# showlab/VideoSwap

Measured on AMD Instinct MI355X. Metric: denoised frames/sec, 16-frame 512x512 clip @ 50 DDIM steps (end to end: inversion + CFG sampling), higher is better.
Workload: dtype f16; 1 GPU; BASELINE.json configs[1]: 16-frame 512x512 clip, SD-1.5 UNet3D + AnimateDiff motion modules, 50-step DDIM inversion (B=1) + 50-step CFG-7.5 DDIM sampling (B=2), 1 clip per GPU per step; launch=eager, parallelism=clip-parallel x1

## Files before the change

videoswap_amd/build.py:

```python
import hashlib
import os
import re
import shutil
import subprocess
import sys
import tempfile
from concurrent.futures import ThreadPoolExecutor

HERE = os.path.dirname(os.path.abspath(__file__))
ROOT = os.path.dirname(HERE)
CSRC = os.path.join(HERE, 'csrc')
LIBDIR = os.path.join(HERE, 'lib')
OBJDIR = os.path.join(LIBDIR, 'obj')
LIB = os.path.join(LIBDIR, 'libvsx.so')
VARIANTS = {}
VARIANT_EXTRA = {}
SOURCES = ['api.cpp', 'comm.cpp', 'options.cpp', 'prof.cpp', 'gemm.hip', 'gemm_pp.hip', 'norm.hip', 'attention.hip', 'attention_bwd.hip', 'elementwise.hip',
           'train.hip', 'dift.hip', 'atlas.hip', 'atlas_edit.hip']
HIPCC = os.environ.get('HIPCC', '/opt/rocm/bin/hipcc')
FLAGS = ['--offload-arch=gfx950', '-O3', '-std=c++17', '-fPIC', '-x', 'hip',
         '-I', os.path.join(ROOT, 'include'), '-I', CSRC, '-Wall', '-Wno-unused-function', '-Wno-division-by-zero',
         '-mllvm', '-amdgpu-mfma-vgpr-form']


def lib_path(variant=None):
    return LIB if not variant else os.path.join(LIBDIR, f'libvsx_{variant}.so')


def _digest(variant=None):
    h = hashlib.sha256()
    swap = VARIANTS[variant] if variant else {}
    names = [n for n in sorted(os.listdir(CSRC)) if n.endswith(('.hip', '.cpp', '.h'))]
    for name in names + ['../../include/vsx.h']:
        with open(os.path.join(CSRC, swap.get(name, name)), 'rb') as f:
            h.update(name.encode() + b'\0' + f.read())
    h.update(' '.join(f.replace(ROOT, '<root>') for f in FLAGS).encode())
    if variant:
        for name in VARIANT_EXTRA.get(variant, []):
            with open(os.path.join(CSRC, name), 'rb') as f:
                h.update(name.encode() + b'\0' + f.read())
        h.update(b'\0variant ' + variant.encode())
    return h.hexdigest()


def source_digest(variant=None):
    return _digest(variant)


_MARKER = b'@vsx-source-digest:'


def built_digest(variant=None):
    path = lib_path(variant)
    if not os.path.exists(path):
        return None
    with open(path, 'rb') as f:
        blob = f.read()
    i = blob.find(_MARKER)
    if i < 0:
        return None
    j = blob.find(b'\0', i)
    return blob[i + len(_MARKER):j].decode(errors='replace')


def _compile(src, digest, variant=None):
    objdir = OBJDIR if not variant else os.path.join(LIBDIR, f'obj_{variant}')
    os.makedirs(objdir, exist_ok=True)
    obj = os.path.join(objdir, src.replace('/', '_') + '.o')
    extra = [f'-DVSX_SOURCE_DIGEST="{digest}"'] if src == 'api.cpp' else []
    path = os.path.join(CSRC, (VARIANTS[variant] if variant else {}).get(src, src))
    cmd = [HIPCC] + FLAGS + extra + ['-c', path, '-o', obj]
    r = subprocess.run(cmd, capture_output=True, text=True)
    if r.returncode != 0:
        raise RuntimeError(f'hipcc failed for {src}:\n{r.stdout}\n{r.stderr}')
    if r.stderr.strip():
        sys.stderr.write(r.stderr)
    return obj


LLVM_BIN = os.environ.get('VSX_LLVM_BIN', '/opt/rocm/lib/llvm/bin')
NO_SCRATCH = ('gemm_pp_kernel', 'gemm_ws320_kernel', 'flash_attn_kernel', 'gemm_kernelILi256E', 'coord_mlp_kernel')


def parse_kernel_notes(text):
    keys = ('vgpr_count', 'agpr_count', 'sgpr_count', 'vgpr_spill_count', 'sgpr_spill_count',
            'private_segment_fixed_size', 'group_segment_fixed_size')
    out, cur = {}, None
    for line in text.splitlines():
        m = re.match(r'^\s+(-\s+)?\.(\w+):\s*(\S.*)?$', line)
        if not m:
            continue
        if m.group(1) and re.match(r'^  - ', line):
            cur = {}
        if cur is None:
            continue
        key, val = m.group(2), (m.group(3) or '').strip()
        if key == 'name' and re.match(r'^    \.name:', line):
            out[val] = cur
        elif key in keys and re.match(r'^  (- |  )\.', line):
            cur[key] = int(val)
    return out


def kernel_resources(lib=None):
    lib = lib or LIB
    objdump, readelf = os.path.join(LLVM_BIN, 'llvm-objdump'), os.path.join(LLVM_BIN, 'llvm-readelf')
    tmp = tempfile.mkdtemp(prefix='vsx_co_')
    try:
        copy = os.path.join(tmp, 'lib.so')
        shutil.copy(lib, copy)
        r = subprocess.run([objdump, '--offloading', copy], capture_output=True, text=True, cwd=tmp)
        if r.returncode != 0:
            raise RuntimeError(f'llvm-objdump --offloading failed:\n{r.stderr}')
        res = {}
        for name in sorted(os.listdir(tmp)):
            if 'gfx950' not in name:
                continue
            r = subprocess.run([readelf, '--notes', os.path.join(tmp, name)], capture_output=True, text=True)
            if r.returncode != 0:
                raise RuntimeError(f'llvm-readelf --notes failed on {name}:\n{r.stderr}')
            res.update(parse_kernel_notes(r.stdout))
        return res
    finally:
        shutil.rmtree(tmp, ignore_errors=True)


def demangle(names):
    filt = shutil.which('c++filt') or shutil.which('llvm-cxxfilt')
    out = []
    if filt and names:
        r = subprocess.run([filt], input='\n'.join(names), capture_output=True, text=True)
        out = r.stdout.splitlines() if r.returncode == 0 else []
    return dict(zip(names, out if len(out) == len(names) else names))


def scratch_offenders(resources, patterns=NO_SCRATCH):
    pretty = demangle(list(resources))
    bad = []
    for name, r in resources.items():
        if not any(p in name for p in patterns):
            continue
        if r.get('vgpr_spill_count', 0) or r.get('private_segment_fixed_size', 0):
            bad.append((pretty[name], r.get('vgpr_spill_count', 0), r.get('private_segment_fixed_size', 0)))
    return sorted(bad)


def check_no_scratch(lib=None):
    res = kernel_resources(lib)
    if not res:
        raise RuntimeError('no kernel metadata found in ' + (lib or LIB))
    bad = scratch_offenders(res)
    if bad:
        raise RuntimeError('kernels that must not use scratch do:\n' + '\n'.join(
            f'  {n}: {s} VGPRs spilled, {b} B private segment' for n, s, b in bad))
    return res


def build(force=False, verbose=True, variant=None):
    os.makedirs(OBJDIR, exist_ok=True)
    lib = lib_path(variant)
    digest = _digest(variant)
    if not force and built_digest(variant) == digest:
        if verbose:
            print(f'[vsx] {lib} is up to date')
# ... 96 lines not shown
```

videoswap_amd/csrc/attention.hip:

```cpp
#include "common.h"
#include "options.h"

#include <type_traits>

namespace {

struct AttnParams {
    const half_t* Q;
    const half_t* K;
    const half_t* VT;
    half_t* O;
    int nq, nk, heads;
    long ldq, ldk, ldvt, ldo;
    long q_bs, k_bs, vt_bs, o_bs;
    int kv_div;
    float scale_log2e;
    float* lse;
    long lse_ld;
};

#ifdef VSX_GEMM_TIMING
__device__ long* g_attn_dbg = nullptr;
#define ASTAMP(i) do { const long t_now = (long)clock64(); t_seg[i] += t_now - t_last; t_last = t_now; } while (0)
#else
#define ASTAMP(i) do { } while (0)
#endif

constexpr int KV_TILE = 64;
constexpr int VSTR = 72;
typedef __attribute__((address_space(3))) void* lds_ptr_t;

template <int D, int QB = 1, bool O16 = false>
__global__ __launch_bounds__(256) void flash_attn_kernel(const AttnParams p) {
    static_assert(!O16 || (QB == 1 && D % 16 != 0 && D <= 48), "16-row O tiles: one query block per wave, a spare padding row");
    constexpr int DK = (D + 15) / 16;
    constexpr int DT = (D + 31) / 32;
    constexpr int CT = (D + 15) / 16;
    constexpr int VROWS = O16 ? CT * 16 : DT * 32;
    constexpr int KSTR = DK * 16 + 8;
    constexpr bool HAS_SPARE = (VROWS > D);
    constexpr int KSPR = KSTR / 8, VSPR = VSTR / 8;
    constexpr int K_UNITS = KV_TILE * KSPR, V_UNITS = D * VSPR;
    constexpr int NKI = (K_UNITS + 255) / 256, NVI = (V_UNITS + 255) / 256;
    constexpr int K_BYTES = KV_TILE * KSTR * 2;
    constexpr int V_BYTES = VROWS * VSTR * 2;
    constexpr int STAGE = K_BYTES + V_BYTES;
    constexpr int OOB_OFF = (int)0x80000000;

    __shared__ __attribute__((aligned(16))) unsigned char smem[2 * STAGE];

    const int tid = threadIdx.x;
    const int lane = tid & 63;
    const int wave = __builtin_amdgcn_readfirstlane(tid >> 6);
    const int l31 = lane & 31, hi = lane >> 5;
    int wg = blockIdx.x;
    {
        const int nwg = gridDim.x, qq = nwg >> 3, rr = nwg & 7;
        const int xcd = wg & 7, local = wg >> 3;
        wg = (xcd < rr ? xcd * (qq + 1) : rr * (qq + 1) + (xcd - rr) * qq) + local;
    }
    constexpr int QTILE = 128 * QB;
    const int qtiles = (p.nq + QTILE - 1) / QTILE;
    const int qt = wg % qtiles;
    const int h = (wg / qtiles) % p.heads;
    const long b = wg / (qtiles * p.heads);
    const long kvb = b / p.kv_div;

    const int q0 = qt * QTILE + wave * (32 * QB) + l31;

    h8 qf[QB][DK];
#pragma unroll
    for (int x = 0; x < QB; ++x) {
        const int q = q0 + 32 * x;
        const bool qok = q < p.nq;
        const half_t* qrow = p.Q + b * p.q_bs + (long)(qok ? q : 0) * p.ldq + h * D;
#pragma unroll
        for (int t = 0; t < DK; ++t) {
            const int d0 = t * 16 + hi * 8;
            qf[x][t] = (qok && d0 < D) ? as_h8(ld16(qrow + d0)) : as_h8(make_uint4(0, 0, 0, 0));
        }
    }

    const half_t* Kb = p.K + kvb * p.k_bs + h * D;
    const half_t* Vb = p.VT + kvb * p.vt_bs + (long)h * D * p.ldvt;
    const __amdgpu_buffer_rsrc_t rsrcK = __builtin_amdgcn_make_buffer_rsrc(
        const_cast<half_t*>(Kb), 0, (int)((((long)p.nk - 1) * p.ldk + D) * 2), 0x00020000);
    const __amdgpu_buffer_rsrc_t rsrcV = __builtin_amdgcn_make_buffer_rsrc(
        const_cast<half_t*>(Vb), 0, (int)((long)D * p.ldvt * 2), 0x00020000);
    int vk[NKI], vv[NVI];
#pragma unroll
    for (int i = 0; i < NKI; ++i) {
        const int u = (wave * NKI + i) * 64 + lane;
        const int row = u / KSPR, slot = u - row * KSPR;
        const int key = (row & ~12) | ((row & 4) << 1) | ((row & 8) >> 1);
        vk[i] = (u < K_UNITS && slot * 8 < D) ? (int)(((long)key * p.ldk + slot * 8) * 2) : OOB_OFF;
    }
#pragma unroll
    for (int i = 0; i < NVI; ++i) {
        const int u = (wave * NVI + i) * 64 + lane;
        const int row = u / VSPR, slot = u - row * VSPR;
        vv[i] = (u < V_UNITS && slot < 8) ? (int)(((long)row * p.ldvt + slot * 8) * 2) : OOB_OFF;
    }
    for (int i = tid; i < 2 * (VROWS - D) * VSTR; i += 256) {
        const int st = i / ((VROWS - D) * VSTR), r = i - st * ((VROWS - D) * VSTR);
        const int row = D + r / VSTR, col = r - (r / VSTR) * VSTR;
        half_t* sv = reinterpret_cast<half_t*>(smem + st * STAGE + K_BYTES);
        sv[row * VSTR + col] = (HAS_SPARE && row == VROWS - 1 && col < KV_TILE) ? (half_t)1.f : (half_t)0.f;
    }

    auto issue = [&](int j0, int stage) {
        unsigned char* sb = smem + stage * STAGE;
        const int soffK = (int)((long)j0 * p.ldk * 2);
        const int soffV = j0 * 2;
// ... 160 lines not shown
                h8 pf[QB];
#pragma unroll
                for (int x = 0; x < QB; ++x) {
#pragma unroll
                    for (int jj = 0; jj < 8; ++jj) pf[x][jj] = (half_t)s[x][kt][8 * s2 + jj];
                }
                const int c0 = kt * 32 + 16 * s2 + 8 * hi;
#pragma unroll
                for (int t = 0; t < DT; ++t) {
                    const h8 vf = *reinterpret_cast<const h8*>(sV + (t * 32 + l31) * VSTR + c0);
#pragma unroll
                    for (int x = 0; x < QB; ++x) o[x][t] = __builtin_amdgcn_mfma_f32_32x32x16_f16(vf, pf[x], o[x][t], 0, 0, 0);
                }
            }
        }
        ASTAMP(5);
        stage ^= 1;
    };
    {
        int j0 = 0;
        for (; j0 + KV_TILE <= p.nk; j0 += KV_TILE) tile(j0, std::false_type{});
        if (j0 < p.nk) tile(j0, std::true_type{});
    }

#ifdef VSX_GEMM_TIMING
    if (lane == 0 && g_attn_dbg) {
        long* o_dbg = g_attn_dbg + ((long)blockIdx.x * 4 + wave) * 6;
        for (int k = 0; k < 6; ++k) o_dbg[k] = t_seg[k];
    }
#endif
    if constexpr (O16) {
        const int l15 = lane & 15, g = lane >> 4;
#pragma unroll
        for (int qt = 0; qt < 2; ++qt) {
            const float den = __shfl(o16[CT - 1][qt][3], 48 + l15, 64);
            const int q = (q0 - l31) + 16 * qt + l15;
            if (q < p.nq) {
                const float inv = 1.0f / den;
                half_t* orow = p.O + b * p.o_bs + (long)q * p.ldo + h * D;
#pragma unroll
                for (int t = 0; t < CT; ++t) {
                    const int c = t * 16 + 4 * g;
                    if (c < D) {
                        h4 pk;
#pragma unroll
                        for (int e = 0; e < 4; ++e) pk[e] = (half_t)(o16[t][qt][e] * inv);
                        *reinterpret_cast<h4*>(orow + c) = pk;
                    }
                }
            }
        }
        return;
    }
#pragma unroll
    for (int x = 0; x < QB; ++x) {
        if (HAS_SPARE) {
            constexpr int reg = 15;
            constexpr int owner_hi = 1;
            const float mine = o[x][DT - 1][reg];
            const float other = __shfl_xor(mine, 32, 64);
            l_i[x] = (hi == owner_hi) ? mine : other;
        }
        const int q = q0 + 32 * x;
        if (q < p.nq) {
            if (p.lse && hi == 0) p.lse[(b * p.heads + h) * p.lse_ld + q] = m_i[x] + __log2f(l_i[x]);
            const float inv = 1.0f / l_i[x];
            half_t* orow = p.O + b * p.o_bs + (long)q * p.ldo + h * D;
#pragma unroll
            for (int t = 0; t < DT; ++t)
#pragma unroll
                for (int g = 0; g < 4; ++g) {
                    const int c = t * 32 + 8 * g + 4 * hi;
                    if (c < D) {
                        h4 pk;
#pragma unroll
                        for (int e = 0; e < 4; ++e) pk[e] = (half_t)(o[x][t][4 * g + e] * inv);
                        *reinterpret_cast<h4*>(orow + c) = pk;
                    }
                }
        }
    }
}

template <int D>
int launch_attn(const AttnParams& p, long nb, hipStream_t stream) {
    if constexpr (D == 40 || D == 80) {
        const long wg2 = ((p.nq + 255) / 256) * (long)p.heads * nb;
        const long force = vsxg::gemm_option("attn_qb");
        if (force == 2 || (force == 0 && D == 80 && wg2 >= 512 && p.nq >= 256)) {
            hipLaunchKernelGGL((flash_attn_kernel<D, 2>), dim3((unsigned)wg2), dim3(256), 0, stream, p);
            return vsx_check_launch("vsx_attention_f16");
        }
    }
    dim3 grid((unsigned)(((p.nq + 127) / 128) * (long)p.heads * nb));
    if constexpr (D == 40) {
        if (p.lse == nullptr && vsxg::gemm_option("attn_o16") != 0) {
            hipLaunchKernelGGL((flash_attn_kernel<D, 1, true>), grid, dim3(256), 0, stream, p);
            return vsx_check_launch("vsx_attention_f16");
        }
    }
    hipLaunchKernelGGL((flash_attn_kernel<D, 1>), grid, dim3(256), 0, stream, p);
    return vsx_check_launch("vsx_attention_f16");
}

struct TempParams {
    const half_t* Q;
    const half_t* K;
    const half_t* V;
    half_t* O;
    int fq, fk, hw, heads, d;
    long ldq, ldkv, ldo;
    float scale;
    int direct_out;
};

__global__ __launch_bounds__(256) void temporal_attn_kernel(const TempParams p) {
    extern __shared__ __attribute__((aligned(16))) unsigned char smem_raw[];
    const int d = p.d, fq = p.fq, fk = p.fk;
    const int wave = threadIdx.x >> 6;
    const size_t slice = (((size_t)(fq + 2 * fk) * d * sizeof(half_t) + (size_t)fq * fk * sizeof(float)) + 15) & ~(size_t)15;
    unsigned char* base = smem_raw + wave * slice;
    half_t* sQ = reinterpret_cast<half_t*>(base);
    half_t* sK = sQ + fq * d;
    half_t* sV = sK + fk * d;
    float* sS = reinterpret_cast<float*>(sV + fk * d);

    const int lane = threadIdx.x & 63;
    const long site = blockIdx.x;
    const int h = min((int)blockIdx.y * 4 + wave, p.heads - 1);
    const long b = blockIdx.z;
    const int dv = d >> 3;

    constexpr int UB = 4;
    for (int i0 = lane; i0 < fq * dv; i0 += 64 * UB) {
        uint4 r[UB];
#pragma unroll
        for (int u = 0; u < UB; ++u) {
            const int i = i0 + 64 * u;
            if (i < fq * dv) {
                const int f = i / dv, c = (i - f * dv) * 8;
                r[u] = ld16(p.Q + ((b * fq + f) * p.hw + site) * p.ldq + h * d + c);
            }
        }
#pragma unroll
        for (int u = 0; u < UB; ++u) {
            const int i = i0 + 64 * u;
            if (i < fq * dv) {
                const int f = i / dv, c = (i - f * dv) * 8;
                st16(sQ + f * d + c, r[u]);
            }
        }
    }
    for (int i0 = lane; i0 < fk * dv; i0 += 64 * UB) {
        uint4 rk[UB], rv[UB];
#pragma unroll
        for (int u = 0; u < UB; ++u) {
            const int i = i0 + 64 * u;
            if (i < fk * dv) {
                const int f = i / dv, c = (i - f * dv) * 8;
                const long row = (b * fk + f) * p.hw + site;
                rk[u] = ld16(p.K + row * p.ldkv + h * d + c);
                rv[u] = ld16(p.V + row * p.ldkv + h * d + c);
            }
        }
#pragma unroll
        for (int u = 0; u < UB; ++u) {
// ... 123 lines not shown
#pragma unroll
    for (int r = 0; r < 16; ++r) {
        const int key = (r & 3) + 4 * ((r >> 2) & 1) + 8 * hi + 16 * (r >> 3);
        const bool v = qok && key >= lo && key < up;
        sc[r] = v ? sc[r] * sl2 : -INFINITY;
        mx = fmaxf(mx, sc[r]);
    }
    mx = fmaxf(mx, __shfl_xor(mx, 32, 64));
    if (mx == -INFINITY) mx = 0.f;
    float sum = 0.f;
#pragma unroll
    for (int r = 0; r < 16; ++r) {
        sc[r] = __builtin_amdgcn_exp2f(sc[r] - mx);
        sum += sc[r];
    }
    sum += __shfl_xor(sum, 32, 64);
    const float inv = sum > 0.f ? 1.0f / sum : 0.f;

    f16v o[DT];
#pragma unroll
    for (int t = 0; t < DT; ++t) o[t] = zero;
#pragma unroll
    for (int s2 = 0; s2 < 2; ++s2) {
        h8 pf;
#pragma unroll
        for (int jj = 0; jj < 8; ++jj) pf[jj] = (half_t)sc[8 * s2 + jj];
#pragma unroll
        for (int t = 0; t < DT; ++t) {
            const h8 vf = *reinterpret_cast<const h8*>(sVT + (t * 32 + l31) * VSTR + vt_col(16 * s2 + 8 * hi, (t * 32 + l31) >> 3));
            o[t] = __builtin_amdgcn_mfma_f32_32x32x16_f16(vf, pf, o[t], 0, 0, 0);
        }
    }
    if (p.direct_out) {
        if (qok) {
            half_t* orow = p.O + ((b * fq + qf_) * p.hw + site) * p.ldo + (long)(head0 + qg) * D;
#pragma unroll
            for (int t = 0; t < DT; ++t)
#pragma unroll
                for (int g4 = 0; g4 < 4; ++g4) {
                    const int c = t * 32 + 8 * g4 + 4 * hi;
                    if (c < D) {
                        h4 pk;
#pragma unroll
                        for (int e = 0; e < 4; ++e) pk[e] = (half_t)(o[t][4 * g4 + e] * inv);
                        *reinterpret_cast<h4*>(orow + c) = pk;
                    }
                }
        }
        return;
    }
    constexpr int OSTR = D + 4;
    static_assert(32 * OSTR <= DT * 32 * VSTR, "the staged output fits the wave's V^T tile");
    static_assert((D / 2 + 2) % 4 == 2, "staged row pitch");
    half_t* sO = sVT;
    __builtin_amdgcn_sched_barrier(0);
#pragma unroll
    for (int t = 0; t < DT; ++t)
#pragma unroll
        for (int g4 = 0; g4 < 4; ++g4) {
            const int c = t * 32 + 8 * g4 + 4 * hi;
            if (c < D) {
                h4 pk;
#pragma unroll
                for (int e = 0; e < 4; ++e) pk[e] = (half_t)(o[t][4 * g4 + e] * inv);
                *reinterpret_cast<h4*>(sO + l31 * OSTR + c) = pk;
            }
        }
    __builtin_amdgcn_sched_barrier(0);
    const int per_frame = G * DV;
    const int total = fq * per_frame;
#pragma unroll
    for (int i = 0; i < NVL; ++i) {
        const int u = lane + 64 * i;
        if (u < total) {
            const int f = u / per_frame, rem = u - f * per_frame;
            const int g = rem / DV, ch = rem - g * DV;
            if (head0 + g < p.heads) {
                const half_t* src = sO + (g * fq + f) * OSTR + ch * 8;
                const h4 lo4 = *reinterpret_cast<const h4*>(src), up4 = *reinterpret_cast<const h4*>(src + 4);
                const h8 v = {lo4[0], lo4[1], lo4[2], lo4[3], up4[0], up4[1], up4[2], up4[3]};
                st16(p.O + ((b * fq + f) * p.hw + site) * p.ldo + (long)(head0 + g) * D + ch * 8, as_u4(v));
            }
        }
    }
}

template <int D>
__global__ __launch_bounds__(256) void temporal_attn_mfma_long_kernel(const TempParams p) {
    constexpr int DK = (D + 15) / 16;
    constexpr int DT = (D + 31) / 32;
    constexpr int DV = D / 8;
    constexpr int VSTR = 40;
    constexpr int NVL = (32 * DV + 63) / 64;
    constexpr int NKB = 4;
    __shared__ __attribute__((aligned(16))) half_t smem[4][DT * 32 * VSTR];

    const int lane = threadIdx.x & 63;
    const int wave = threadIdx.x >> 6;
    const int l31 = lane & 31, hi = lane >> 5;
    const int fq = p.fq, fk = p.fk;
    const int G = 32 / fq;
    const int nkb = (fk + 31) >> 5;
    const long site = blockIdx.x;
    const long b = blockIdx.z;
    const int head0 = ((int)blockIdx.y * 4 + wave) * G;
    if (head0 >= p.heads) return;
    half_t* sVT = smem[wave];

    const int qg = l31 / fq, qf_ = l31 - qg * fq;
    const bool qok = qg < G && head0 + qg < p.heads;
    const half_t* qptr = p.Q + ((b * fq + qf_) * p.hw + site) * p.ldq + (long)(head0 + qg) * D + hi * 8;
    h8 qb[DK];
#pragma unroll
    for (int t = 0; t < DK; ++t)
        qb[t] = (qok && t * 16 + hi * 8 < D) ? as_h8(ld16(qptr + t * 16)) : as_h8(make_uint4(0, 0, 0, 0));

    const f16v zero = {0.f, 0.f, 0.f, 0.f, 0.f, 0.f, 0.f, 0.f, 0.f, 0.f, 0.f, 0.f, 0.f, 0.f, 0.f, 0.f};
    f16v sc[NKB];
#pragma unroll
    for (int kb = 0; kb < NKB; ++kb) sc[kb] = zero;
    const int krow = (l31 & ~12) | ((l31 & 4) << 1) | ((l31 & 8) >> 1);
    for (int g = 0; g < G; ++g) {
        if (head0 + g >= p.heads) break;
#pragma unroll
        for (int kb = 0; kb < NKB; ++kb) {
            if (kb >= nkb) continue;
            const int key = kb * 32 + krow;
            const half_t* kptr = p.K + ((b * fk + key) * p.hw + site) * p.ldkv + (long)(head0 + g) * D + hi * 8;
            f16v tile = zero;
#pragma unroll
            for (int t = 0; t < DK; ++t) {
                const h8 ka = (key < fk && t * 16 + hi * 8 < D) ? as_h8(ld16(kptr + t * 16)) : as_h8(make_uint4(0, 0, 0, 0));
                tile = __builtin_amdgcn_mfma_f32_32x32x16_f16(ka, qb[t], tile, 0, 0, 0);
            }
            if (g == qg) sc[kb] = tile;
        }
    }

    const float sl2 = p.scale * 1.44269504088896340736f;
    float mx = -INFINITY;
#pragma unroll
    for (int kb = 0; kb < NKB; ++kb)
#pragma unroll
        for (int r = 0; r < 16; ++r) {
            const int key = kb * 32 + (r & 3) + 4 * ((r >> 2) & 1) + 8 * hi + 16 * (r >> 3);
            const bool v = qok && kb < nkb && key < fk;
            sc[kb][r] = v ? sc[kb][r] * sl2 : -INFINITY;
            mx = fmaxf(mx, sc[kb][r]);
        }
    mx = fmaxf(mx, __shfl_xor(mx, 32, 64));
    if (mx == -INFINITY) mx = 0.f;
    float sum = 0.f;
#pragma unroll
    for (int kb = 0; kb < NKB; ++kb)
#pragma unroll
        for (int r = 0; r < 16; ++r) {
            sc[kb][r] = __builtin_amdgcn_exp2f(sc[kb][r] - mx);
            sum += sc[kb][r];
        }
    sum += __shfl_xor(sum, 32, 64);
    const float inv = sum > 0.f ? 1.0f / sum : 0.f;

    f16v o[DT];
#pragma unroll
    for (int t = 0; t < DT; ++t) o[t] = zero;
    for (int g = 0; g < G; ++g) {
        if (head0 + g >= p.heads) break;
#pragma unroll
        for (int kb = 0; kb < NKB; ++kb) {
            if (kb >= nkb) continue;
            uint4 raw[NVL];
#pragma unroll
            for (int i = 0; i < NVL; ++i) {
                const int u = lane + 64 * i;
                const int kk = u / DV, ch = u - kk * DV;
                const int key = kb * 32 + kk;
                raw[i] = (u < 32 * DV && key < fk)
                             ? ld16(p.V + ((b * fk + key) * p.hw + site) * p.ldkv + (long)(head0 + g) * D + ch * 8)
                             : make_uint4(0, 0, 0, 0);
            }
#pragma unroll
            for (int i = 0; i < NVL; ++i) {
                const int u = lane + 64 * i;
                if (u < 32 * DV) {
                    const int kk = u / DV, ch = u - kk * DV;
                    const h8 v = as_h8(raw[i]);
#pragma unroll
                    for (int e = 0; e < 8; ++e) sVT[(ch * 8 + e) * VSTR + vt_col(kk, ch)] = v[e];
                }
            }
#pragma unroll
            for (int s2 = 0; s2 < 2; ++s2) {
                h8 pf;
#pragma unroll
                for (int jj = 0; jj < 8; ++jj) pf[jj] = g == qg ? (half_t)sc[kb][8 * s2 + jj] : (half_t)0.f;
#pragma unroll
                for (int t = 0; t < DT; ++t) {
                    const h8 vf = *reinterpret_cast<const h8*>(sVT + (t * 32 + l31) * VSTR + vt_col(16 * s2 + 8 * hi, (t * 32 + l31) >> 3));
                    o[t] = __builtin_amdgcn_mfma_f32_32x32x16_f16(vf, pf, o[t], 0, 0, 0);
                }
            }
        }
    }
    if (qok) {
        half_t* orow = p.O + ((b * fq + qf_) * p.hw + site) * p.ldo + (long)(head0 + qg) * D;
#pragma unroll
        for (int t = 0; t < DT; ++t)
#pragma unroll
            for (int g4 = 0; g4 < 4; ++g4) {
                const int c = t * 32 + 8 * g4 + 4 * hi;
                if (c < D) {
                    h4 pk;
#pragma unroll
                    for (int e = 0; e < 4; ++e) pk[e] = (half_t)(o[t][4 * g4 + e] * inv);
                    *reinterpret_cast<h4*>(orow + c) = pk;
                }
            }
    }
}

template <int D>
int launch_temporal_mfma_long(const TempParams& p, long B, hipStream_t stream) {
    const int G = 32 / p.fq;
    const int groups = (p.heads + G - 1) / G;
    dim3 grid((unsigned)p.hw, (unsigned)((groups + 3) / 4), (unsigned)B);
    hipLaunchKernelGGL((temporal_attn_mfma_long_kernel<D>), grid, dim3(256), 0, stream, p);
    return vsx_check_launch("vsx_temporal_attention_f16");
}

template <int D>
int launch_temporal_mfma(const TempParams& p, long B, hipStream_t stream) {
    const int G = 32 / (p.fq > p.fk ? p.fq : p.fk);
    const int groups = (p.heads + G - 1) / G;
    dim3 grid((unsigned)p.hw, (unsigned)((groups + 3) / 4), (unsigned)B);
    hipLaunchKernelGGL((temporal_attn_mfma_kernel<D>), grid, dim3(256), 0, stream, p);
    return vsx_check_launch("vsx_temporal_attention_f16");
}

}

#ifdef VSX_GEMM_TIMING
extern "C" int vsx_attn_debug_buffer(void* buf) {
    return hipMemcpyToSymbol(HIP_SYMBOL(g_attn_dbg), &buf, sizeof(buf)) == hipSuccess ? 0 : 1;
}
#endif

static int attention_fwd(const void* Q, const void* K, const void* VT, void* O, float* lse, int64_t lse_ld, int64_t nb, int64_t heads,
                         int64_t nq, int64_t nk, int64_t d, int64_t ldq, int64_t ldk, int64_t ldvt, int64_t ldo, int64_t q_bs,
                         int64_t k_bs, int64_t vt_bs, int64_t o_bs, int64_t kv_div, float scale, vsx_stream_t stream_);

extern "C" int vsx_attention_f16(const void* Q, const void* K, const void* VT, void* O, int64_t nb, int64_t heads,
                                 int64_t nq, int64_t nk, int64_t d, int64_t ldq, int64_t ldk, int64_t ldvt,
                                 int64_t ldo, int64_t q_bs, int64_t k_bs, int64_t vt_bs, int64_t o_bs,
                                 int64_t kv_div, float scale, vsx_stream_t stream) {
    return attention_fwd(Q, K, VT, O, nullptr, 0, nb, heads, nq, nk, d, ldq, ldk, ldvt, ldo, q_bs, k_bs, vt_bs, o_bs, kv_div, scale,
                         stream);
}

extern "C" int vsx_attention_lse_f16(const void* Q, const void* K, const void* VT, void* O, float* lse, int64_t lse_ld,
                                     int64_t nb, int64_t heads, int64_t nq, int64_t nk, int64_t d, int64_t ldq, int64_t ldk,
                                     int64_t ldvt, int64_t ldo, int64_t q_bs, int64_t k_bs, int64_t vt_bs, int64_t o_bs,
                                     int64_t kv_div, float scale, vsx_stream_t stream) {
    VSX_REQUIRE(lse != nullptr && lse_ld >= nq, VSX_E_BADSHAPE, "attention_lse: lse buffer / row length");
    return attention_fwd(Q, K, VT, O, lse, lse_ld, nb, heads, nq, nk, d, ldq, ldk, ldvt, ldo, q_bs, k_bs, vt_bs, o_bs, kv_div, scale,
                         stream);
}

static int attention_fwd(const void* Q, const void* K, const void* VT, void* O, float* lse, int64_t lse_ld, int64_t nb, int64_t heads,
                         int64_t nq, int64_t nk, int64_t d, int64_t ldq, int64_t ldk, int64_t ldvt, int64_t ldo, int64_t q_bs,
                         int64_t k_bs, int64_t vt_bs, int64_t o_bs, int64_t kv_div, float scale, vsx_stream_t stream_) {
    hipStream_t stream = (hipStream_t)stream_;
    VSX_REQUIRE(Q && K && VT && O, VSX_E_BADSHAPE, "attention: null tensor");
    if (nb == 0 || nq == 0) return VSX_OK;
    VSX_REQUIRE(nb > 0 && heads > 0 && nq > 0 && nk > 0 && kv_div > 0, VSX_E_BADSHAPE, "attention: bad sizes");
    VSX_REQUIRE(nb <= 65535 && heads <= 65535, VSX_E_BADSHAPE, "attention: nb/heads exceed grid limits");
    VSX_REQUIRE(vsx_aligned16(Q) && vsx_aligned16(K) && vsx_aligned16(VT) && vsx_aligned16(O), VSX_E_BADSHAPE,
                "attention: tensors must be 16-byte aligned");
    VSX_REQUIRE(ldq % 8 == 0 && ldk % 8 == 0 && ldvt % 8 == 0 && ldo % 4 == 0, VSX_E_BADSHAPE,
                "attention: row strides must be multiples of 8 (ldo: 4)");
    VSX_REQUIRE(q_bs % 8 == 0 && k_bs % 8 == 0 && vt_bs % 8 == 0 && o_bs % 4 == 0, VSX_E_BADSHAPE,
                "attention: batch strides must be multiples of 8");
    VSX_REQUIRE(ldvt >= ((nk + 7) / 8) * 8, VSX_E_BADSHAPE, "attention: ldvt (%ld) < round_up(nk=%ld, 8)", (long)ldvt,
                (long)nk);
    AttnParams p;
    p.Q = (const half_t*)Q; p.K = (const half_t*)K; p.VT = (const half_t*)VT; p.O = (half_t*)O;
    p.nq = (int)nq; p.nk = (int)nk; p.heads = (int)heads;
    p.ldq = ldq; p.ldk = ldk; p.ldvt = ldvt; p.ldo = ldo;
    p.q_bs = q_bs; p.k_bs = k_bs; p.vt_bs = vt_bs; p.o_bs = o_bs;
    p.kv_div = (int)kv_div;
    p.scale_log2e = scale * 1.44269504088896340736f;
    p.lse = lse;
    p.lse_ld = lse_ld;
    switch (d) {
        case 8: return launch_attn<8>(p, nb, stream);
        case 16: return launch_attn<16>(p, nb, stream);
        case 32: return launch_attn<32>(p, nb, stream);
        case 40: return launch_attn<40>(p, nb, stream);
        case 64: return launch_attn<64>(p, nb, stream);
        case 80: return launch_attn<80>(p, nb, stream);
        case 128: return launch_attn<128>(p, nb, stream);
        case 160: return launch_attn<160>(p, nb, stream);
        default: return vsx_fail(VSX_E_UNSUPPORTED, "attention: head dim %ld not in {8,16,32,40,64,80,128,160}", (long)d);
    }
}

extern "C" int vsx_temporal_attention_f16(const void* Q, const void* K, const void* V, void* O, int64_t B, int64_t fq,
                                          int64_t fk, int64_t hw, int64_t heads, int64_t d, int64_t ldq, int64_t ldkv,
                                          int64_t ldo, float scale, vsx_stream_t stream) {
    VSX_REQUIRE(Q && K && V && O, VSX_E_BADSHAPE, "temporal_attention: null tensor");
    if (B == 0 || hw == 0) return VSX_OK;
    VSX_REQUIRE(B > 0 && fq > 0 && fk > 0 && hw > 0 && heads > 0 && d > 0, VSX_E_BADSHAPE, "temporal_attention: bad sizes");
    VSX_REQUIRE(d % 8 == 0 && ldq % 8 == 0 && ldkv % 8 == 0 && ldo % 8 == 0, VSX_E_BADSHAPE,
                "temporal_attention: d and row strides must be multiples of 8");
    VSX_REQUIRE(vsx_aligned16(Q) && vsx_aligned16(K) && vsx_aligned16(V) && vsx_aligned16(O), VSX_E_BADSHAPE,
                "temporal_attention: tensors must be 16-byte aligned");
    VSX_REQUIRE(B <= 65535 && heads <= 65535, VSX_E_BADSHAPE, "temporal_attention: grid limits");
    TempParams p;
    p.Q = (const half_t*)Q; p.K = (const half_t*)K; p.V = (const half_t*)V; p.O = (half_t*)O;
    p.fq = (int)fq; p.fk = (int)fk; p.hw = (int)hw; p.heads = (int)heads; p.d = (int)d;
    p.ldq = ldq; p.ldkv = ldkv; p.ldo = ldo; p.scale = scale;
    p.direct_out = vsxg::gemm_option("temporal_out") == 1 ? 1 : 0;
    if (fq <= 32 && fk <= 32) {
        if (d == 40) return launch_temporal_mfma<40>(p, B, (hipStream_t)stream);
        if (d == 80) return launch_temporal_mfma<80>(p, B, (hipStream_t)stream);
        if (d == 160) return launch_temporal_mfma<160>(p, B, (hipStream_t)stream);
    } else if (fq <= 32 && fk <= 128) {
        if (d == 40) return launch_temporal_mfma_long<40>(p, B, (hipStream_t)stream);
        if (d == 80) return launch_temporal_mfma_long<80>(p, B, (hipStream_t)stream);
        if (d == 160) return launch_temporal_mfma_long<160>(p, B, (hipStream_t)stream);
    }
    const size_t slice = (((size_t)(fq + 2 * fk) * d * sizeof(half_t) + (size_t)fq * fk * sizeof(float)) + 15) & ~(size_t)15;
    const size_t smem = 4 * slice;
    VSX_REQUIRE(smem <= 160 * 1024, VSX_E_UNSUPPORTED, "temporal_attention: %zu bytes of LDS needed (> 160 KiB)", smem);
    static size_t smem_attr = 64 * 1024;
    if (smem > smem_attr) {
        hipError_t e = hipFuncSetAttribute(reinterpret_cast<const void*>(&temporal_attn_kernel),
                                           hipFuncAttributeMaxDynamicSharedMemorySize, 160 * 1024);
        if (e != hipSuccess) return vsx_fail(VSX_E_LAUNCH, "temporal_attention: hipFuncSetAttribute: %s", hipGetErrorString(e));
        smem_attr = 160 * 1024;
    }
    dim3 grid((unsigned)hw, (unsigned)((heads + 3) / 4), (unsigned)B);
    hipLaunchKernelGGL(temporal_attn_kernel, grid, dim3(256), smem, (hipStream_t)stream, p);
    return vsx_check_launch("vsx_temporal_attention_f16");
}
```

videoswap_amd/csrc/options.cpp:

```cpp
#include "options.h"

#include <stdlib.h>
#include <string.h>

#include "common.h"

namespace vsxg {
namespace {
struct Option { const char* name; const char* env; long value; bool init; };
Option g_options[] = {{"gemm_pp", "VSX_GEMM_PP", 1, false}, {"pp_sched", "VSX_PP_SCHED", 0, false},
                      {"tile_tune", "VSX_TUNE_TILE", 0, false}, {"xcd_walk", "VSX_XCD_WALK", 1, false},
                      {"attn_qb", "VSX_ATTN_QB", 0, false}, {"temporal_out", "VSX_TEMPORAL_OUT", 0, false},
                      {"attn_o16", "VSX_ATTN_O16", 0, false}, {"gn_fuse", "VSX_GN_FUSE", 0, false},
                      {"gemm_ws", "VSX_GEMM_WS", 1, false}, {"ws_waves", "VSX_WS_WAVES", 10, false}};
Option* find_option(const char* name) {
    for (auto& o : g_options)
        if (strcmp(o.name, name) == 0) {
            if (!o.init) {
                const char* e = getenv(o.env);
                if (e) o.value = atol(e);
                o.init = true;
            }
            return &o;
        }
    return nullptr;
}
}
long gemm_option(const char* name) {
    Option* o = find_option(name);
    return o ? o->value : 0;
}
}

extern "C" int vsx_set_option(const char* name, int64_t value) {
    auto* o = name ? vsxg::find_option(name) : nullptr;
    if (!o) return vsx_fail(VSX_E_BADSHAPE, "vsx_set_option: unknown option '%s'", name ? name : "(null)");
    o->value = (long)value;
    return VSX_OK;
}
```

Baseline: 4.149 frames/s.

## Add persistent resident-KV cross-attention and streaming temporal attention kernels

Adds a persistent attention kernel for short-key attention (nk<=128, e.g. cross-attention to text tokens). It keeps K/V in registers across query blocks, prefetches the next Q tile, and gets the softmax denominator from a ones row in the spare V^T tile. Also adds a grid-stride temporal attention kernel that prefetches the next problem's Q/K/V while computing the current one and reads V through LDS transpose loads. Both are on by default through new options. Together they aim to cut launch and reload overhead and hide memory latency in the many small attention problems. The cost is more register pressure and more complex index walking.

```diff
diff --git a/videoswap_amd/build.py b/videoswap_amd/build.py
--- a/videoswap_amd/build.py
+++ b/videoswap_amd/build.py
@@ -79,7 +79,8 @@
 
 
 LLVM_BIN = os.environ.get('VSX_LLVM_BIN', '/opt/rocm/lib/llvm/bin')
-NO_SCRATCH = ('gemm_pp_kernel', 'gemm_ws320_kernel', 'flash_attn_kernel', 'gemm_kernelILi256E', 'coord_mlp_kernel')
+NO_SCRATCH = ('gemm_pp_kernel', 'gemm_ws320_kernel', 'flash_attn_kernel', 'gemm_kernelILi256E', 'coord_mlp_kernel',
+              'attn_resident_kernel', 'temporal_attn_stream_kernel')
 
 
 def parse_kernel_notes(text):
diff --git a/videoswap_amd/csrc/attention.hip b/videoswap_amd/csrc/attention.hip
--- a/videoswap_amd/csrc/attention.hip
+++ b/videoswap_amd/csrc/attention.hip
@@ -29,6 +29,20 @@
 constexpr int KV_TILE = 64;
 constexpr int VSTR = 72;
 typedef __attribute__((address_space(3))) void* lds_ptr_t;
+
+int device_cus(int* n) {
+    static int n_cu = 0;
+    if (n_cu == 0) {
+        int dev = 0;
+        hipDeviceProp_t prop;
+        if (hipGetDevice(&dev) != hipSuccess || hipGetDeviceProperties(&prop, dev) != hipSuccess)
+            return vsx_fail(VSX_E_LAUNCH, "attention: cannot query the device");
+        n_cu = prop.multiProcessorCount > 0 ? prop.multiProcessorCount : 256;
+    }
+    *n = n_cu;
+    return VSX_OK;
+}
+
 
 template <int D, int QB = 1, bool O16 = false>
 __global__ __launch_bounds__(256) void flash_attn_kernel(const AttnParams p) {
@@ -355,6 +369,234 @@
     }
 }
 
+template <int D, int HG, int NKB>
+__global__ __launch_bounds__(HG * 64) void attn_resident_kernel(const AttnParams p, const int nb, const int qblocks, const long nunits) {
+    constexpr int DK = (D + 15) / 16;
+    constexpr int DT = (D + 31) / 32;
+    constexpr int NT = HG * 64;
+    constexpr int RW = HG * D;
+    constexpr int CH = RW / 8;
+    constexpr int NQL = (32 * CH + NT - 1) / NT;
+    constexpr int QP = RW + 8;
+    constexpr int OP = RW + 4;
+    constexpr int DEN_T = D / 32, DEN_R = (D % 32) / 2;
+    static_assert(D % 8 == 0 && D % 32 != 0, "row D of the last O^T tile is spare: it carries the denominator");
+    static_assert((CH & 1) == 0 && (RW / 2 + 2) % 4 == 2, "staged row pitches");
+    __shared__ __attribute__((aligned(16))) half_t sQ[32 * QP];
+    __shared__ __attribute__((aligned(16))) half_t sO[32 * OP];
+
+    const int tid = threadIdx.x;
+    const int lane = tid & 63;
+    const int wave = __builtin_amdgcn_readfirstlane(tid >> 6);
+    const int l31 = lane & 31, hi = lane >> 5;
+
+    struct Walk { long u; int qb, b, hgrp, kvb, brem; };
+    const long per = (nunits + gridDim.x - 1) / gridDim.x;
+    Walk cw;
+    cw.u = (long)blockIdx.x * per;
+    const long uend = cw.u + per < nunits ? cw.u + per : nunits;
+    if (cw.u >= uend) return;
+    cw.qb = (int)(cw.u % qblocks); cw.b = (int)((cw.u / qblocks) % nb); cw.hgrp = (int)(cw.u / ((long)qblocks * nb));
+    cw.kvb = cw.b / p.kv_div; cw.brem = cw.b - cw.kvb * p.kv_div;
+    Walk fw = cw;
+    auto advance = [&](Walk& w) __attribute__((always_inline)) -> bool {
+        bool new_kv = false;
+        ++w.u;
+        if (++w.qb == qblocks) {
+            w.qb = 0;
+            ++w.b;
+            if (++w.brem == p.kv_div) { w.brem = 0; ++w.kvb; new_kv = true; }
+            if (w.b == nb) { w.b = 0; w.brem = 0; w.kvb = 0; ++w.hgrp; new_kv = true; }
+        }
+        return new_kv;
+    };
+
+    int qrow[NQL], qdst[NQL];
+    unsigned qoff[NQL], ooff[NQL];
+#pragma unroll
+    for (int i = 0; i < NQL; ++i) {
+        const int c = tid + NT * i;
+        const int row = c / CH, ch = c - row * CH;
+        qrow[i] = c < 32 * CH ? row : 32;
+        qdst[i] = row * QP + ch * 8;
+        qoff[i] = (unsigned)((long)row * p.ldq + ch * 8);
+        ooff[i] = (unsigned)((long)row * p.ldo + ch * 8);
+    }
+    const int krow = (l31 & ~12) | ((l31 & 4) << 1) | ((l31 & 8) >> 1);
+    const f16v zero = {0.f, 0.f, 0.f, 0.f, 0.f, 0.f, 0.f, 0.f, 0.f, 0.f, 0.f, 0.f, 0.f, 0.f, 0.f, 0.f};
+
+    h8 ka[NKB][DK], va[DT][2 * NKB];
+    auto load_kv = [&](const int kb_, const int h) __attribute__((always_inline)) {
+        const half_t* Kb = p.K + (long)kb_ * p.k_bs + (long)h * D;
+        const half_t* Vb = p.VT + (long)kb_ * p.vt_bs + (long)h * D * p.ldvt;
+#pragma unroll
+        for (int kb = 0; kb < NKB; ++kb)
+#pragma unroll
+            for (int t = 0; t < DK; ++t) {
+                const int key = kb * 32 + krow;
+                ka[kb][t] = (key < p.nk && t * 16 + hi * 8 < D) ? as_h8(ld16(Kb + (long)key * p.ldk + t * 16 + hi * 8))
+                                                                : as_h8(make_uint4(0, 0, 0, 0));
+            }
+#pragma unroll
+        for (int t = 0; t < DT; ++t)
+#pragma unroll
+            for (int ks = 0; ks < 2 * NKB; ++ks) {
+                const int c = t * 32 + l31, key0 = ks * 16 + 8 * hi;
+                h8 v = as_h8(make_uint4(0, 0, 0, 0));
+                if (c < D && key0 < p.nk) {
+                    v = as_h8(ld16(Vb + (long)c * p.ldvt + key0));
+#pragma unroll
+                    for (int e = 0; e < 8; ++e)
+                        if (key0 + e >= p.nk) v[e] = (half_t)0.f;
+                } else if (c == D) {
+#pragma unroll
+                    for (int e = 0; e < 8; ++e) v[e] = (half_t)1.f;
+                }
+                va[t][ks] = v;
+            }
+    };
+    auto issue_q = [&](const Walk& w, uint4 (&qraw)[NQL]) __attribute__((always_inline)) {
+        const half_t* qbase = p.Q + (long)w.b * p.q_bs + (long)w.qb * 32 * p.ldq + (long)w.hgrp * RW;
+        const int rows = min(32, p.nq - w.qb * 32);
+#pragma unroll
+        for (int i = 0; i < NQL; ++i) qraw[i] = qrow[i] < rows ? ld16(qbase + qoff[i]) : make_uint4(0, 0, 0, 0);
+    };
+
+    auto block = [&](uint4 (&qraw)[NQL]) __attribute__((always_inline)) -> bool {
+        half_t* obase = p.O + (long)cw.b * p.o_bs + (long)cw.qb * 32 * p.ldo + (long)cw.hgrp * RW;
+        const int rows = min(32, p.nq - cw.qb * 32);
+#pragma unroll
+        for (int i = 0; i < NQL; ++i)
+            if (qrow[i] < 32) st16(sQ + qdst[i], qraw[i]);
+        if (fw.u < uend) {
+            issue_q(fw, qraw);
+            advance(fw);
+        }
+        __syncthreads();
+
+        h8 qf[DK];
+#pragma unroll
+        for (int t = 0; t < DK; ++t)
+            qf[t] = t * 16 + hi * 8 < D ? *reinterpret_cast<const h8*>(sQ + l31 * QP + wave * D + t * 16 + hi * 8)
+                                        : as_h8(make_uint4(0, 0, 0, 0));
+        f16v s[NKB];
+#pragma unroll
+        for (int kb = 0; kb < NKB; ++kb)
+#pragma unroll
+            for (int t = 0; t < DK; ++t)
+                s[kb] = __builtin_amdgcn_mfma_f32_32x32x16_f16(ka[kb][t], qf[t], t == 0 ? zero : s[kb], 0, 0, 0);
+
+#pragma unroll
+        for (int kb = 0; kb < NKB; ++kb)
+            if (kb * 32 + 32 > p.nk) {
+#pragma unroll
+                for (int r = 0; r < 16; ++r) {
+                    const int key = kb * 32 + (r & 3) + 4 * ((r >> 2) & 1) + 8 * hi + 16 * (r >> 3);
+                    if (key >= p.nk) s[kb][r] = -INFINITY;
+                }
+            }
+        float mx = -INFINITY;
+#pragma unroll
+        for (int kb = 0; kb < NKB; ++kb)
+#pragma unroll
+            for (int s2 = 0; s2 < 2; ++s2)
+                if (32 * kb + 16 * s2 < p.nk) {
+#pragma unroll
+                    for (int jj = 0; jj < 8; jj += 2) mx = fmaxf(fmaxf(mx, s[kb][8 * s2 + jj]), s[kb][8 * s2 + jj + 1]);
+                }
+        mx = fmaxf(mx, __shfl_xor(mx, 32, 64)) * p.scale_log2e;
+        {
+            const vsx_f2 sc2 = {p.scale_log2e, p.scale_log2e}, nm2 = {-mx, -mx};
+#pragma unroll
+            for (int kb = 0; kb < NKB; ++kb)
+#pragma unroll
+                for (int s2 = 0; s2 < 2; ++s2)
+                    if (32 * kb + 16 * s2 < p.nk) {
+#pragma unroll
+                        for (int r = 8 * s2; r < 8 * s2 + 8; r += 2) {
+                            const vsx_f2 t = vsx_f2{s[kb][r], s[kb][r + 1]} * sc2 + nm2;
+                            s[kb][r] = __builtin_amdgcn_exp2f(t[0]);
+                            s[kb][r + 1] = __builtin_amdgcn_exp2f(t[1]);
+                        }
+                    }
+        }
+
+        f16v o[DT];
+#pragma unroll
+        for (int t = 0; t < DT; ++t) o[t] = zero;
+#pragma unroll
+        for (int kb = 0; kb < NKB; ++kb)
+#pragma unroll
+            for (int s2 = 0; s2 < 2; ++s2)
+                if (32 * kb + 16 * s2 < p.nk) {
+                    h8 pf;
+#pragma unroll
+                    for (int jj = 0; jj < 8; ++jj) pf[jj] = (half_t)s[kb][8 * s2 + jj];
+#pragma unroll
+                    for (int t = 0; t < DT; ++t) o[t] = __builtin_amdgcn_mfma_f32_32x32x16_f16(va[t][2 * kb + s2], pf, o[t], 0, 0, 0);
+                }
+        const float inv = 1.0f / __shfl(o[DEN_T][DEN_R], l31, 64);
+
+#pragma unroll
+        for (int t = 0; t < DT; ++t)
+#pragma unroll
+            for (int g4 = 0; g4 < 4; ++g4) {
+                const int c = t * 32 + 8 * g4 + 4 * hi;
+                if (c < D) {
+                    h4 pk;
+#pragma unroll
+                    for (int e = 0; e < 4; ++e) pk[e] = (half_t)(o[t][4 * g4 + e] * inv);
+                    *reinterpret_cast<h4*>(sO + l31 * OP + wave * D + c) = pk;
+                }
+            }
+        __syncthreads();
+#pragma unroll
+        for (int i = 0; i < NQL; ++i)
+            if (qrow[i] < rows) {
+                const half_t* src = sO + qdst[i] - 4 * qrow[i];
+                const h4 lo4 = *reinterpret_cast<const h4*>(src), up4 = *reinterpret_cast<const h4*>(src + 4);
+                const h8 v = {lo4[0], lo4[1], lo4[2], lo4[3], up4[0], up4[1], up4[2], up4[3]};
+                st16(obase + ooff[i], as_u4(v));
+            }
+        const bool new_kv = advance(cw);
+        if (cw.u >= uend) return false;
+        if (new_kv) load_kv(cw.kvb, cw.hgrp * HG + wave);
+        return true;
+    };
+
+    uint4 qa[NQL];
+    issue_q(fw, qa);
+    advance(fw);
+    load_kv(cw.kvb, cw.hgrp * HG + wave);
+    while (block(qa)) {}
+}
+
+template <int D, int HG>
+int launch_attn_resident(const AttnParams& p, long nb, hipStream_t stream) {
+    const int qblocks = (p.nq + 31) / 32;
+    const long nunits = (long)(p.heads / HG) * nb * qblocks;
+    int n_cu = 0;
+    if (int rc = device_cus(&n_cu)) return rc;
+    const dim3 grid((unsigned)(nunits < n_cu ? nunits : n_cu));
+    if constexpr (D == 40 && HG == 8) {
+        hipLaunchKernelGGL((attn_resident_kernel<D, HG, 3>), grid, dim3(HG * 64), 0, stream, p, (int)nb, qblocks, nunits);
+    } else if constexpr (D == 40) {
+        hipLaunchKernelGGL((attn_resident_kernel<D, HG, 4>), grid, dim3(HG * 64), 0, stream, p, (int)nb, qblocks, nunits);
+    } else if (p.nk <= 96) {
+        hipLaunchKernelGGL((attn_resident_kernel<D, HG, 3>), grid, dim3(HG * 64), 0, stream, p, (int)nb, qblocks, nunits);
+    } else {
+        hipLaunchKernelGGL((attn_resident_kernel<D, HG, 4>), grid, dim3(HG * 64), 0, stream, p, (int)nb, qblocks, nunits);
+    }
+    return vsx_check_launch("vsx_attention_f16");
+}
+
+inline int attn_resident_heads(const AttnParams& p, int d) { return d == 40 ? (p.nk <= 96 ? 8 : 4) : d == 80 ? 4 : 0; }
+inline bool attn_resident_ok(const AttnParams& p, int d) {
+    const int hg = attn_resident_heads(p, d);
+    return hg != 0 && p.lse == nullptr && p.nk <= 128 && p.heads % hg == 0 && p.ldo % 8 == 0 && p.o_bs % 8 == 0 &&
+           p.ldq < (1L << 26) && p.ldo < (1L << 26);
+}
+
 template <int D>
 int launch_attn(const AttnParams& p, long nb, hipStream_t stream) {
     if constexpr (D == 40 || D == 80) {
@@ -644,6 +886,182 @@
                 st16(p.O + ((b * fq + f) * p.hw + site) * p.ldo + (long)(head0 + g) * D + ch * 8, as_u4(v));
             }
         }
+    }
+}
+
+constexpr int tr_pitch(const int cols) {
+    int pitch = (cols + 31) / 32 * 32;
+    while (pitch % 128 != 32 && pitch % 128 != 96) pitch += 32;
+    return pitch;
+}
+
+typedef __fp16 vsx_fp16x4 __attribute__((__vector_size__(4 * sizeof(__fp16))));
+__device__ __forceinline__ h4 lds_read_tr16(const half_t* p) {
+    return __builtin_bit_cast(h4, __builtin_amdgcn_ds_read_tr16_b64_v4f16((__attribute__((address_space(3))) vsx_fp16x4*)p));
+}
+
+template <int D>
+__global__ __launch_bounds__(256, (D <= 40 ? 4 : D <= 80 ? 2 : 1)) void temporal_attn_stream_kernel(const TempParams p, const int groups, const long nprob) {
+    constexpr int DK = (D + 15) / 16;
+    constexpr int DT = (D + 31) / 32;
+    constexpr int DV = D / 8;
+    constexpr int NVL = (32 * DV + 63) / 64;
+    constexpr int PITCH = tr_pitch(DT * 32);
+    constexpr int OSTR = D + 4;
+    constexpr int SLICE = 32 * (PITCH > OSTR ? PITCH : OSTR);
+    constexpr int NONE = 1 << 20;
+    static_assert((D / 2 + 2) % 4 == 2, "staged row pitch");
+    __shared__ __attribute__((aligned(16))) half_t smem[4][SLICE];
+
+    const int lane = threadIdx.x & 63;
+    const int wave = __builtin_amdgcn_readfirstlane(threadIdx.x >> 6);
+    const int l31 = lane & 31, hi = lane >> 5;
+    const int fq = p.fq, fk = p.fk, heads = p.heads;
+    const int G = 32 / max(fq, fk);
+    half_t* sV = smem[wave];
+
+    long w = (long)blockIdx.x * 4 + wave;
+    if (w >= nprob) return;
+    const long wstride = (long)gridDim.x * 4;
+    int hg = (int)(w % groups), site = (int)((w / groups) % p.hw), b = (int)(w / ((long)groups * p.hw));
+    const int s_hg = (int)(wstride % groups), s_site = (int)((wstride / groups) % p.hw), s_b = (int)(wstride / ((long)groups * p.hw));
+
+    unsigned voff[NVL], ooff[NVL];
+    int vdst[NVL], vg[NVL], osrc[NVL], og[NVL];
+    {
+        const int per_frame = G * DV, total = fq * per_frame;
+#pragma unroll
+        for (int i = 0; i < NVL; ++i) {
+            const int u = lane + 64 * i;
+            const int key = u / DV, ch = u - key * DV;
+            const int g = key / fk, f = key - g * fk;
+            vdst[i] = u < 32 * DV ? key * PITCH + ch * 8 : -1;
+            vg[i] = (u < 32 * DV && g < G) ? g : NONE;
+            voff[i] = (unsigned)((long)f * p.hw * p.ldkv + (long)g * D + ch * 8);
+            const int fo = u / per_frame, rem = u - fo * per_frame;
+            const int go = rem / DV, co = rem - go * DV;
+            og[i] = u < total ? go : NONE;
+            osrc[i] = (go * fq + fo) * OSTR + co * 8;
+            ooff[i] = (unsigned)((long)fo * p.hw * p.ldo + (long)go * D + co * 8);
+        }
+    }
+    const int krow = (l31 & ~12) | ((l31 & 4) << 1) | ((l31 & 8) >> 1);
+    const int kg = krow / fk, kf_ = krow - kg * fk;
+    const int qg = l31 / fq, qf_ = l31 - qg * fq;
+    const int kgh = kg < G ? kg : NONE, qgh = qg < G ? qg : NONE;
+    const unsigned koff = (unsigned)((long)kf_ * p.hw * p.ldkv + (long)kg * D + hi * 8);
+    const unsigned qoff = (unsigned)((long)qf_ * p.hw * p.ldq + (long)qg * D + hi * 8);
+    const int lo = qg * fk, up = lo + fk;
+    const float sl2 = p.scale * 1.44269504088896340736f;
+    const half_t* trbase = sV + (8 * hi + ((l31 >> 2) & 3)) * PITCH + (l31 >> 4) * 16 + (l31 & 3) * 4;
+    const f16v zero = {0.f, 0.f, 0.f, 0.f, 0.f, 0.f, 0.f, 0.f, 0.f, 0.f, 0.f, 0.f, 0.f, 0.f, 0.f, 0.f};
+
+    auto issue = [&](const int bb, const int ss, const int head0, uint4 (&raw)[NVL], h8 (&ka)[DK], h8 (&qb)[DK]) {
+        const half_t* vbase = p.V + ((long)bb * fk * p.hw + ss) * p.ldkv + (long)head0 * D;
+        const half_t* kbase = p.K + ((long)bb * fk * p.hw + ss) * p.ldkv + (long)head0 * D;
+        const half_t* qbase = p.Q + ((long)bb * fq * p.hw + ss) * p.ldq + (long)head0 * D;
+#pragma unroll
+        for (int i = 0; i < NVL; ++i) raw[i] = head0 + vg[i] < heads ? ld16(vbase + voff[i]) : make_uint4(0, 0, 0, 0);
+        const bool kok = head0 + kgh < heads, qok = head0 + qgh < heads;
+#pragma unroll
+        for (int t = 0; t < DK; ++t) {
+            const bool in = t * 16 + hi * 8 < D;
+            ka[t] = (kok && in) ? as_h8(ld16(kbase + koff + t * 16)) : as_h8(make_uint4(0, 0, 0, 0));
+            qb[t] = (qok && in) ? as_h8(ld16(qbase + qoff + t * 16)) : as_h8(make_uint4(0, 0, 0, 0));
+        }
+    };
+
+    uint4 raw[NVL];
+    h8 ka[DK], qb[DK];
+    issue(b, site, hg * G, raw, ka, qb);
+    for (;;) {
+        const int head0 = hg * G;
+        const bool qok = head0 + qgh < heads;
+        half_t* obase = p.O + ((long)b * fq * p.hw + site) * p.ldo + (long)head0 * D;
+#pragma unroll
+        for (int i = 0; i < NVL; ++i)
+            if (vdst[i] >= 0) st16(sV + vdst[i], raw[i]);
+        w += wstride;
+        const bool more = w < nprob;
+        hg += s_hg;
+        if (hg >= groups) { hg -= groups; ++site; }
+        site += s_site;
+        if (site >= p.hw) { site -= p.hw; ++b; }
+        b += s_b;
+        uint4 raw_n[NVL];
+        h8 ka_n[DK], qb_n[DK];
+        if (more) issue(b, site, hg * G, raw_n, ka_n, qb_n);
+        __builtin_amdgcn_sched_barrier(0);
+
+        f16v sc = zero;
+#pragma unroll
+        for (int t = 0; t < DK; ++t) sc = __builtin_amdgcn_mfma_f32_32x32x16_f16(ka[t], qb[t], t == 0 ? zero : sc, 0, 0, 0);
+
+        float mx = -INFINITY;
+#pragma unroll
+        for (int r = 0; r < 16; ++r) {
+            const int key = (r & 3) + 4 * ((r >> 2) & 1) + 8 * hi + 16 * (r >> 3);
+            const bool v = qok && key >= lo && key < up;
+            sc[r] = v ? sc[r] * sl2 : -INFINITY;
+            mx = fmaxf(mx, sc[r]);
+        }
+        mx = fmaxf(mx, __shfl_xor(mx, 32, 64));
+        if (mx == -INFINITY) mx = 0.f;
+        float sum = 0.f;
+#pragma unroll
+        for (int r = 0; r < 16; ++r) {
+            sc[r] = __builtin_amdgcn_exp2f(sc[r] - mx);
+            sum += sc[r];
+        }
+        sum += __shfl_xor(sum, 32, 64);
+        const float inv = sum > 0.f ? 1.0f / sum : 0.f;
+
+        f16v o[DT];
+#pragma unroll
+        for (int t = 0; t < DT; ++t) o[t] = zero;
+#pragma unroll
+        for (int s2 = 0; s2 < 2; ++s2) {
+            h8 pf;
+#pragma unroll
+            for (int jj = 0; jj < 8; ++jj) pf[jj] = (half_t)sc[8 * s2 + jj];
+#pragma unroll
+            for (int t = 0; t < DT; ++t) {
+                const h4 v0 = lds_read_tr16(trbase + (16 * s2) * PITCH + t * 32);
+                const h4 v1 = lds_read_tr16(trbase + (16 * s2 + 4) * PITCH + t * 32);
+                const h8 vfrag = {v0[0], v0[1], v0[2], v0[3], v1[0], v1[1], v1[2], v1[3]};
+                o[t] = __builtin_amdgcn_mfma_f32_32x32x16_f16(vfrag, pf, o[t], 0, 0, 0);
+            }
+        }
+
+        half_t* sO = sV;
+        __builtin_amdgcn_sched_barrier(0);
+#pragma unroll
+        for (int t = 0; t < DT; ++t)
+#pragma unroll
+            for (int g4 = 0; g4 < 4; ++g4) {
+                const int c = t * 32 + 8 * g4 + 4 * hi;
+                if (c < D) {
+                    h4 pk;
+#pragma unroll
+                    for (int e = 0; e < 4; ++e) pk[e] = (half_t)(o[t][4 * g4 + e] * inv);
+                    *reinterpret_cast<h4*>(sO + l31 * OSTR + c) = pk;
+                }
+            }
+        __builtin_amdgcn_sched_barrier(0);
+#pragma unroll
+        for (int i = 0; i < NVL; ++i)
+            if (head0 + og[i] < heads) {
+                const half_t* src = sO + osrc[i];
+                const h4 lo4 = *reinterpret_cast<const h4*>(src), up4 = *reinterpret_cast<const h4*>(src + 4);
+                const h8 v = {lo4[0], lo4[1], lo4[2], lo4[3], up4[0], up4[1], up4[2], up4[3]};
+                st16(obase + ooff[i], as_u4(v));
+            }
+        if (!more) break;
+        __builtin_amdgcn_sched_barrier(0);
+#pragma unroll
+        for (int i = 0; i < NVL; ++i) raw[i] = raw_n[i];
+#pragma unroll
+        for (int t = 0; t < DK; ++t) { ka[t] = ka_n[t]; qb[t] = qb_n[t]; }
     }
 }
 
@@ -796,6 +1214,18 @@
     const int groups = (p.heads + G - 1) / G;
     dim3 grid((unsigned)p.hw, (unsigned)((groups + 3) / 4), (unsigned)B);
     hipLaunchKernelGGL((temporal_attn_mfma_kernel<D>), grid, dim3(256), 0, stream, p);
+    return vsx_check_launch("vsx_temporal_attention_f16");
+}
+
+template <int D>
+int launch_temporal_stream(const TempParams& p, long B, long per_cu, hipStream_t stream) {
+    const int G = 32 / (p.fq > p.fk ? p.fq : p.fk);
+    const int groups = (p.heads + G - 1) / G;
+    const long nprob = B * p.hw * groups;
+    int n_cu = 0;
+    if (int rc = device_cus(&n_cu)) return rc;
+    const long cap = (long)n_cu * (per_cu > 1 ? per_cu : 2), need = (nprob + 3) / 4;
+    hipLaunchKernelGGL((temporal_attn_stream_kernel<D>), dim3((unsigned)(need < cap ? need : cap)), dim3(256), 0, stream, p, groups, nprob);
     return vsx_check_launch("vsx_temporal_attention_f16");
 }
 
@@ -853,6 +1283,17 @@
     p.scale_log2e = scale * 1.44269504088896340736f;
     p.lse = lse;
     p.lse_ld = lse_ld;
+    const long resident = vsxg::gemm_option("attn_resident");
+    bool take = resident != 0 && attn_resident_ok(p, (int)d);
+    if (take && resident == 1) {
+        int n_cu = 0;
+        if (int rc = device_cus(&n_cu)) return rc;
+        take = (heads / attn_resident_heads(p, (int)d)) * nb * ((nq + 31) / 32) >= 8L * n_cu;
+    }
+    if (take) {
+        if (d == 80) return launch_attn_resident<80, 4>(p, nb, stream);
+        return attn_resident_heads(p, 40) == 8 ? launch_attn_resident<40, 8>(p, nb, stream) : launch_attn_resident<40, 4>(p, nb, stream);
+    }
     switch (d) {
         case 8: return launch_attn<8>(p, nb, stream);
         case 16: return launch_attn<16>(p, nb, stream);
@@ -883,6 +1324,13 @@
     p.ldq = ldq; p.ldkv = ldkv; p.ldo = ldo; p.scale = scale;
     p.direct_out = vsxg::gemm_option("temporal_out") == 1 ? 1 : 0;
     if (fq <= 32 && fk <= 32) {
+        const long streams = vsxg::gemm_option("temporal_stream");
+        const int64_t ldmax = ldq > ldkv ? (ldq > ldo ? ldq : ldo) : (ldkv > ldo ? ldkv : ldo);
+        if (streams != 0 && !p.direct_out && 32 * hw * ldmax < ((int64_t)1 << 31)) {
+            if (d == 40) return launch_temporal_stream<40>(p, B, streams, (hipStream_t)stream);
+            if (d == 80) return launch_temporal_stream<80>(p, B, streams, (hipStream_t)stream);
+            if (d == 160 && streams > 1) return launch_temporal_stream<160>(p, B, streams, (hipStream_t)stream);
+        }
         if (d == 40) return launch_temporal_mfma<40>(p, B, (hipStream_t)stream);
         if (d == 80) return launch_temporal_mfma<80>(p, B, (hipStream_t)stream);
         if (d == 160) return launch_temporal_mfma<160>(p, B, (hipStream_t)stream);
diff --git a/videoswap_amd/csrc/options.cpp b/videoswap_amd/csrc/options.cpp
--- a/videoswap_amd/csrc/options.cpp
+++ b/videoswap_amd/csrc/options.cpp
@@ -12,7 +12,8 @@
                       {"tile_tune", "VSX_TUNE_TILE", 0, false}, {"xcd_walk", "VSX_XCD_WALK", 1, false},
                       {"attn_qb", "VSX_ATTN_QB", 0, false}, {"temporal_out", "VSX_TEMPORAL_OUT", 0, false},
                       {"attn_o16", "VSX_ATTN_O16", 0, false}, {"gn_fuse", "VSX_GN_FUSE", 0, false},
-                      {"gemm_ws", "VSX_GEMM_WS", 1, false}, {"ws_waves", "VSX_WS_WAVES", 10, false}};
+                      {"gemm_ws", "VSX_GEMM_WS", 1, false}, {"ws_waves", "VSX_WS_WAVES", 10, false},
+                      {"temporal_stream", "VSX_TEMPORAL_STREAM", 1, false}, {"attn_resident", "VSX_ATTN_RESIDENT", 1, false}};
 Option* find_option(const char* name) {
     for (auto& o : g_options)
         if (strcmp(o.name, name) == 0) {
```

Measured after the change: 4.146 frames/s. No clear change (-0.1%).
